# holo-routing/holo

Measured on NVIDIA H100. Metric: SPF recomputations/sec (10k-node LSDB), higher is better.
Workload: dtype u32

## Files before the change

holo_b200/csrc/spf_quad.cuh:

```cuda
#pragma once
#include <cstdint>
#include <cuda_runtime.h>

#include "spf_kernel.cuh"

namespace hspf {

constexpr uint32_t kJsInvalid = 8u;
constexpr uint32_t kJsInternal = 16u;
constexpr uint32_t kJsNarrow = 32u;
constexpr int kQMaxRoot = 64;

struct QuadDev {
    uint32_t NQ, NIQ, shift, isteps;
    const uint4 *fq;
    const uint32_t *fcont;
    const uint16_t *slot_of;
    const uint16_t *vert_of;
    const uint4 *iq;
    const uint2 *imeta;
    const uint32_t *fpos;
    const uint32_t *ipos;
};

struct QuadLayout {
    uint32_t dist, queue, ring, cont, h0, ecmp, elist, total;
    uint32_t qcap;
    uint32_t mhops;
    uint32_t mcap;
};

struct QuadArgs {
    DevGraph g;
    QuadDev q;
    QuadLayout lay;
    uint32_t n_jobs;
    const uint32_t *roots;
    const uint32_t *ov_off;
    const uint32_t *ov_edge;
    const uint32_t *ov_cost;
    uint32_t *out_dist;
    uint16_t *out_hops;
    uint32_t *out_fp;
    uint16_t *out_npar;
    uint64_t *out_nh;
    uint32_t *out_status;
    uint32_t *job_counter;
    uint32_t sub_rounds;
    uint32_t narrow;
    uint32_t n_peers;
    long long peer_delta[7];
    uint32_t *done;
    uint32_t done_chunk;
    unsigned long long *prof;
};

inline QuadLayout make_quad_layout(uint32_t V, uint32_t NQ, uint32_t qcap, uint32_t threads) {
    QuadLayout L{};
    auto al = [](size_t x) { return (uint32_t)((x + 15) / 16 * 16); };
    const uint32_t nbv = (V + 31) / 32, nbw = (NQ / 32 + 1u) & ~1u;
    const uint32_t Vp = (V + 4 * threads - 1) / (4 * threads) * (4 * threads);
    uint32_t o = 0;
    L.dist = o; o += al((size_t)NQ * 4);
    L.queue = o; o += al((size_t)qcap * 4);
    L.elist = al((size_t)Vp * 4);
    if (L.elist + al((size_t)V * 2) > o) o = L.elist + al((size_t)V * 2);
    L.ring = o; o += al((size_t)4 * nbw * 4);
    L.cont = o; o += al((size_t)nbw * 4);
    L.h0 = o; o += al((size_t)nbv * 4);
    L.ecmp = o; o += al((size_t)nbv * 4);
    L.total = o;
    L.qcap = qcap;
    if (L.cont >= L.elist + al((size_t)Vp * 2)) {
        L.mhops = L.cont - Vp * 2;
        L.mcap = (L.mhops - L.elist) / 2;
    }
    return L;
}

constexpr uint32_t kQuadThreads = 512;
constexpr uint32_t kQuadQcap = 2048;

inline size_t quad_smem_bytes(const QuadLayout &L) { return (size_t)L.total + 2048; }

struct QSmall {
    uint32_t cnt[2];
    uint32_t wake;
    uint32_t status;
    uint32_t job;
    uint32_t n_ov, sh;
    uint32_t ov_edge[kMaxOv], ov_cost[kMaxOv];
    uint32_t ov_fq[kMaxOv], ov_iq[kMaxOv];
    uint32_t n_roottab, root_rb, n_atoms;
    uint32_t mbad;
    uint16_t seed_of[16];
    uint32_t rt_target[kQMaxRoot], rt_base[kQMaxRoot], rt_cost[kQMaxRoot];
};

#define HSPF_QMARK(k)                                                            \
    do {                                                                         \
        if (a.prof && tid == 0) {                                                \
            const long long now_ = clock64();                                    \
            a.prof[(size_t)blockIdx.x * 16 + (k)] += (unsigned long long)(now_ - t_mark); \
            t_mark = now_;                                                       \
        }                                                                        \
    } while (0)

template <int T, bool kOv>
__global__ void __launch_bounds__(T, 3) spf_quad_kernel(const QuadArgs a) {
    extern __shared__ __align__(16) uint8_t qsm[];
    __shared__ QSmall S;

    const DevGraph &g = a.g;
    const QuadDev &Q = a.q;
    const QuadLayout &L = a.lay;
    const uint32_t V = g.V, NQ = Q.NQ, NBW = NQ >> 5, nbv = (V + 31) >> 5;
    const uint32_t NBWp = (NBW + 1u) & ~1u;
    const uint32_t tid = threadIdx.x, lane = tid & 31;
    const uint32_t qcap = L.qcap;

    uint32_t *dist = reinterpret_cast<uint32_t *>(qsm + L.dist);
    uint32_t *queue = reinterpret_cast<uint32_t *>(qsm + L.queue);
    uint32_t *ring = reinterpret_cast<uint32_t *>(qsm + L.ring);
    uint32_t *cont_s = reinterpret_cast<uint32_t *>(qsm + L.cont);
    uint32_t *h0bm = reinterpret_cast<uint32_t *>(qsm + L.h0);
    uint32_t *ecmpbm = reinterpret_cast<uint32_t *>(qsm + L.ecmp);
    uint32_t *word = dist;
    uint16_t *elist = reinterpret_cast<uint16_t *>(qsm + L.elist);

    long long t_mark = clock64();

    for (uint32_t w = tid; w < NBWp; w += T) cont_s[w] = (w < NBW) ? Q.fcont[w] : 0u;
    auto is_hop = [&](uint32_t v) -> bool { return (__ldg(&g.vflags[v]) & kVfHop) != 0; };
    const uint32_t Vp = (V + 4 * T - 1) / (4 * T) * (4 * T);
    const uint32_t U = g.reject_above + 1u ? g.reject_above + 1u : kInf;

    for (;;) {
        __syncthreads();
        if (tid == 0) S.job = atomicAdd(a.job_counter, 1u);
        __syncthreads();
        const uint32_t job = S.job;
        if (job >= a.n_jobs) break;
        const uint32_t root = a.roots[job];
        uint32_t n_ov_raw = 0;
        if (kOv && a.ov_off) n_ov_raw = a.ov_off[job + 1] - a.ov_off[job];
        if (root >= V || n_ov_raw > (uint32_t)kMaxOv) {
            if (tid == 0) {
                a.out_status[job] = kJsInvalid;
                for (uint32_t k = 0; k < (a.narrow ? a.n_peers : 0u); ++k)
                    *reinterpret_cast<uint32_t *>(reinterpret_cast<char *>(&a.out_status[job]) + a.peer_delta[k]) = kJsInvalid;
                if (a.done) { __threadfence(); atomicAdd(&a.done[job / a.done_chunk], 1u); }
            }
            continue;
        }
        const size_t jo = (size_t)job * V;
        const bool narrow = a.narrow != 0;
        uint32_t *o_dist = a.out_dist + jo;
        uint16_t *o_hops = a.out_hops + jo;
        uint32_t *o_fp = a.out_fp + jo;
        uint16_t *o_npar = a.out_npar + jo;
        uint64_t *o_nh = a.out_nh + jo;
        uint16_t *o_dist16 = reinterpret_cast<uint16_t *>(a.out_dist) + jo;
        uint16_t *o_fp16 = reinterpret_cast<uint16_t *>(a.out_fp) + jo;
        uint16_t *o_nh16 = reinterpret_cast<uint16_t *>(a.out_nh) + jo;
        const uint32_t n_peers = narrow ? a.n_peers : 0u;
        auto peer_push_row = [&](uint16_t *row) {
            char *src = reinterpret_cast<char *>(row);
            const size_t bytes = (size_t)V * 2;
            const size_t head = (16 - (reinterpret_cast<uintptr_t>(src) & 15)) & 15;
            const size_t h = head < bytes ? head : bytes;
            const size_t n16 = (bytes - h) / 16, tail0 = h + n16 * 16;
            for (size_t i = tid; i < n16; i += T) {
                const uint4 val = __ldcg(reinterpret_cast<const uint4 *>(src + h) + i);
                for (uint32_t k = 0; k < n_peers; ++k)
                    reinterpret_cast<uint4 *>(src + h + a.peer_delta[k])[i] = val;
            }
            auto push16 = [&](size_t o) {
                const uint16_t val = __ldcg(reinterpret_cast<const uint16_t *>(src + o));
                for (uint32_t k = 0; k < n_peers; ++k) *reinterpret_cast<uint16_t *>(src + o + a.peer_delta[k]) = val;
            };
            for (size_t o = (size_t)tid * 2; o < h; o += (size_t)T * 2) push16(o);
            for (size_t o = tail0 + (size_t)tid * 2; o < bytes; o += (size_t)T * 2) push16(o);
        };
        auto ld_fp = [&](uint32_t v) -> uint32_t {
            if (narrow) { const uint32_t f = __ldcg(&o_fp16[v]); return f == 0xFFFFu ? kInf : f; }
            return __ldcg(&o_fp[v]);
        };
        auto ld_dist = [&](uint32_t v) -> uint32_t {
            if (narrow) { const uint32_t d = __ldcg(&o_dist16[v]); return d == 0xFFFFu ? kInf : d; }
            return __ldcg(&o_dist[v]);
        };

        {
            uint4 *d4 = reinterpret_cast<uint4 *>(dist);
            const uint4 inf4 = make_uint4(U, U, U, U);
            for (uint32_t i = tid; i < NQ / 4; i += T) d4[i] = inf4;
            for (uint32_t i = tid; i < 4 * NBWp; i += T) ring[i] = 0;
            for (uint32_t w = tid; w < nbv; w += T) { h0bm[w] = 0; ecmpbm[w] = 0; }
        }
        if (tid == 0) {
            S.status = 0;
            S.cnt[0] = 0;
            S.cnt[1] = 0;
            S.wake = 0;
            S.n_ov = n_ov_raw;
            S.sh = Q.shift;
        }
        __syncthreads();
        if (kOv && tid < n_ov_raw) {
            const uint32_t e = a.ov_edge[a.ov_off[job] + tid];
            const uint32_t c = a.ov_cost[a.ov_off[job] + tid];
            if (e >= g.E) {
                atomicOr(&S.status, kJsInvalid);
                S.ov_edge[tid] = kInf; S.ov_cost[tid] = kInf; S.ov_fq[tid] = kInf; S.ov_iq[tid] = kInf;
            } else {
                S.ov_edge[tid] = e;
                S.ov_cost[tid] = c;
                S.ov_fq[tid] = Q.fpos[e];
                S.ov_iq[tid] = Q.ipos[e];
                const uint32_t tail = Q.vert_of[Q.fpos[e] >> 2];
                if (c == 0 && (g.vflags[tail] & kVfHop)) atomicOr(&S.status, kJsOrder);
                if (c != kInf) {
                    uint32_t sh = Q.shift;
                    while (sh < 31 && (3ull << sh) < (unsigned long long)c) ++sh;
                    atomicMax(&S.sh, sh);
                }
            }
        }
        const uint32_t rs = Q.slot_of[root];
        if (tid == 0) {
            dist[rs] = 0;
            ring[(rs >> 5) << 2] = 1u << (rs & 31);
        }
        __syncthreads();
        const uint32_t n_ov = kOv ? S.n_ov : 0u;
        auto ov_cost_of = [&](uint32_t e, uint32_t c) -> uint32_t {
            for (uint32_t k = 0; k < n_ov; ++k)
                if (S.ov_edge[k] == e) c = S.ov_cost[k];
            return c;
        };
        if (tid == 32 % T) {
            const uint32_t rb = g.row[root], re = g.row[root + 1];
            uint32_t nt = 0, nextbase = re - rb;
            for (uint32_t e = rb; e < re; ++e) {
                const uint2 ec = g.edge[e];
                const uint32_t h = ec.x;
                if (!(g.vflags[h] & kVfHop)) {
                    if (nt < (uint32_t)kQMaxRoot) {
                        S.rt_target[nt] = h;
                        S.rt_base[nt] = nextbase;
                        S.rt_cost[nt] = ov_cost_of(e, ec.y);
                        ++nt;
                    } else {
                        atomicOr(&S.status, kJsTooManyAtoms);
                    }
                    nextbase += g.row[h + 1] - g.row[h];
                }
            }
            S.n_roottab = nt;
            S.root_rb = rb;
            if (nextbase > 64u) { atomicOr(&S.status, kJsTooManyAtoms); nextbase = 64u; }
            S.n_atoms = nextbase;
        }
        __syncthreads();
        HSPF_QMARK(0);

        const uint32_t sh = kOv ? S.sh : Q.shift;
        {
            auto relax = [&](uint32_t q, uint32_t first, uint32_t du, const uint4 &r4) {
                uint32_t hs[4] = {r4.x & 0xFFFFu, r4.y & 0xFFFFu, r4.z & 0xFFFFu, r4.w & 0xFFFFu};
                uint32_t cs[4] = {r4.x >> 16, r4.y >> 16, r4.z >> 16, r4.w >> 16};
                if (kOv) {
                    for (uint32_t k = 0; k < n_ov; ++k) {
                        const uint32_t fp_ = S.ov_fq[k];
                        if ((fp_ >> 2) != q) continue;
                        const uint32_t c = S.ov_cost[k];
#pragma unroll
                        for (int j = 0; j < 4; ++j)
                            if ((fp_ & 3u) == (uint32_t)j) {
                                if (c == kInf) { hs[j] = first; cs[j] = 0xFFFFu; } else cs[j] = c;
                            }
                    }
                }
                uint32_t dh[4];
#pragma unroll
                for (int j = 0; j < 4; ++j) dh[j] = dist[hs[j]];
#pragma unroll
                for (int j = 0; j < 4; ++j) {
                    const uint32_t nd = kOv ? sat_add(du, cs[j]) : du + cs[j];
                    if (nd < dh[j]) {
                        const uint32_t old = atomicMin(&dist[hs[j]], nd);
                        if (old > nd) atomicOr(&ring[((hs[j] >> 5) << 2) + ((nd >> sh) & 3u)], 1u << (hs[j] & 31));
                    }
                }
            };
            constexpr uint32_t kWarps_ = T / 32;
            const uint32_t warp = tid >> 5;
            const uint32_t cw = min(32u, (NBWp + kWarps_ - 1) / kWarps_);
            const uint32_t nchunks = (NBWp + cw - 1) / cw;
            const uint32_t sub_rounds = a.sub_rounds;
            auto pick = [&](uint32_t t, uint32_t incl, uint32_t bits, uint32_t meta, uint32_t C) -> uint32_t {
                uint32_t lo = 0;
#pragma unroll
                for (uint32_t step = 16; step >= 1; step >>= 1) {
                    const uint32_t v = __shfl_sync(0xffffffffu, incl, lo + step - 1);
                    if (v <= t) lo += step;
                }
                lo &= 31u;
                const uint32_t ob = __shfl_sync(0xffffffffu, bits, lo);
                const uint32_t om = __shfl_sync(0xffffffffu, meta, lo);
                const uint32_t oc = __shfl_sync(0xffffffffu, C, lo);
                uint32_t k = t - (om & 0xFFFFu), pos = 0, cc;
                cc = __popc(ob & 0xFFFFu); if (k >= cc) { k -= cc; pos = 16; }
                cc = __popc((ob >> pos) & 0xFFu); if (k >= cc) { k -= cc; pos += 8; }
                cc = __popc((ob >> pos) & 0xFu); if (k >= cc) { k -= cc; pos += 4; }
                cc = __popc((ob >> pos) & 0x3u); if (k >= cc) { k -= cc; pos += 2; }
                cc = (ob >> pos) & 1u; if (k >= cc) pos += 1;
                pos &= 31u;
                const uint32_t fb = 31u - __clz((~oc & ((2u << pos) - 1u)) | 1u);
                const uint32_t qb = (om >> 16) * 32;
                return (qb + pos) | ((qb + fb) << 16);
            };
            uint32_t cur = 0, empties = 0;
            bool bucket_work = false;
            for (uint32_t guard = 0;; ++guard) {
                if (guard > (1u << 24)) { if (tid == 0) atomicOr(&S.status, kJsInternal); break; }
                uint32_t *bm = ring + (cur & 3u);
                int claimed = 0;
                for (uint32_t sr = 0; sr < sub_rounds; ++sr) {
                    for (uint32_t c = warp; c < nchunks; c += kWarps_) {
                        const uint32_t w = c * cw + lane;
                        const bool mine = lane < cw && w < NBWp;
                        uint32_t bits = mine ? *reinterpret_cast<volatile uint32_t *>(&bm[w << 2]) : 0u;
                        if (!__any_sync(0xffffffffu, bits != 0)) continue;
                        claimed = 1;
                        uint32_t C = 0;
                        if (bits) {
                            bits = atomicExch(&bm[w << 2], 0u);
                            C = cont_s[w];
                            uint32_t m = bits;
                            while ((m = (m << 1) & C) != 0) bits |= m;
                        }
                        const uint32_t cnt = __popc(bits);
                        uint32_t incl = cnt;
#pragma unroll
                        for (int o = 1; o < 32; o <<= 1) {
                            const uint32_t t = __shfl_up_sync(0xffffffffu, incl, o);
                            if ((int)lane >= o) incl += t;
                        }
                        const uint32_t n = __shfl_sync(0xffffffffu, incl, 31);
                        const uint32_t meta = (incl - cnt) | (w << 16);
                        if (a.prof && lane == 0) atomicAdd(&a.prof[(size_t)blockIdx.x * 16 + 12], (unsigned long long)n);
                        for (uint32_t t0 = 0; t0 < n; t0 += 64) {
                            const uint32_t ta = t0 + lane, tb = ta + 32;
                            const bool hb = t0 + 32 < n;
                            const uint32_t e0 = pick(ta, incl, bits, meta, C);
                            const uint32_t e1 = hb ? pick(tb, incl, bits, meta, C) : 0u;
                            const uint32_t du0 = (ta < n) ? dist[e0 >> 16] : kInf;
                            const uint32_t du1 = (hb && tb < n) ? dist[e1 >> 16] : kInf;
                            const bool l0 = (du0 >> sh) == cur, l1 = (du1 >> sh) == cur;
                            uint4 r0 = make_uint4(0u, 0u, 0u, 0u), r1 = r0;
                            if (l0) r0 = __ldg(&Q.fq[e0 & 0xFFFFu]);
                            if (l1) r1 = __ldg(&Q.fq[e1 & 0xFFFFu]);
                            if (l0) relax(e0 & 0xFFFFu, e0 >> 16, du0, r0);
                            if (l1) relax(e1 & 0xFFFFu, e1 >> 16, du1, r1);
                        }
                    }
                }
                if (a.prof && tid == 0) a.prof[(size_t)blockIdx.x * 16 + 7] += 1;
                if (__syncthreads_or(claimed)) { bucket_work = true; continue; }
                if (bucket_work) empties = 0;
                else if (++empties == 4) break;
                bucket_work = false;
                ++cur;
            }
        }
        HSPF_QMARK(1);

        if (tid < S.n_roottab) {
            const uint32_t h = S.rt_target[tid], c = S.rt_cost[tid];
            if (c < U && dist[Q.slot_of[h]] == c) atomicOr(&h0bm[h >> 5], 1u << (h & 31));
        }
        __syncthreads();
        auto hops0 = [&](uint32_t u) -> bool { return u == root || ((h0bm[u >> 5] >> (u & 31)) & 1u); };

        const uint32_t n_atoms = S.n_atoms;
        uint32_t seed_v = kInf;
        if (tid < n_atoms) {
            const uint32_t atom = tid, rdeg = g.row[root + 1] - S.root_rb;
            uint32_t e = kInf, u = root;
            if (atom < rdeg) {
                e = S.root_rb + atom;
            } else {
                for (uint32_t k = 0; k < S.n_roottab; ++k) {
                    const uint32_t N = S.rt_target[k], nb = S.rt_base[k];
                    if (atom < nb || atom >= nb + (g.row[N + 1] - g.row[N])) continue;
                    bool first = true;
                    for (uint32_t q = 0; q < k; ++q) first = first && S.rt_target[q] != N;
                    if (first && hops0(N)) { u = N; e = g.row[N] + (atom - nb); }
                    break;
                }
            }
            if (e != kInf) {
                const uint2 ec = g.edge[e];
                const uint32_t c = kOv ? ov_cost_of(e, ec.y) : ec.y;
                const uint32_t du = dist[Q.slot_of[u]], dh = dist[Q.slot_of[ec.x]];
                if (du < U && dh < U && c != kInf && sat_add(du, c) == dh &&
                    !((g.flags & kGfNoHopTargetNoNh) && !is_hop(ec.x)))
                    seed_v = ec.x;
            }
        }

        {
            uint32_t sat_flag = 0, narrow_flag = 0;
            const uint32_t NIQ = Q.NIQ, isteps = Q.isteps;
            auto pull = [&](uint32_t i, const uint2 &m, const uint4 &r4, uint32_t &dv, uint32_t &cnt, uint32_t &bd, uint32_t &bs) {
                const uint32_t sv = (m.x != 0xFFFFFFFFu) ? (m.x & 0xFFFFu) : 0u;
                dv = dist[sv];
                uint32_t su[4] = {r4.x & 0xFFFFu, r4.y & 0xFFFFu, r4.z & 0xFFFFu, r4.w & 0xFFFFu};
                uint32_t cs[4] = {r4.x >> 16, r4.y >> 16, r4.z >> 16, r4.w >> 16};
                if (kOv) {
                    for (uint32_t k = 0; k < n_ov; ++k) {
                        const uint32_t ip_ = S.ov_iq[k];
                        if ((ip_ >> 2) != i) continue;
                        const uint32_t c = S.ov_cost[k];
#pragma unroll
                        for (int j = 0; j < 4; ++j)
                            if ((ip_ & 3u) == (uint32_t)j) {
                                if (c == kInf) { su[j] = sv; cs[j] = 0xFFFFu; } else cs[j] = c;
                            }
                    }
                }
                uint32_t du[4];
#pragma unroll
                for (int j = 0; j < 4; ++j) du[j] = dist[su[j]];
                cnt = 0; bd = kInf; bs = kInf;
#pragma unroll
                for (int j = 0; j < 4; ++j) {
                    const uint32_t nd = kOv ? sat_add(du[j], cs[j]) : du[j] + cs[j];
                    const bool ok = du[j] < U && nd == dv;
                    const bool better = ok && (du[j] < bd || (du[j] == bd && su[j] < bs));
                    cnt += ok ? 1u : 0u;
                    bd = better ? du[j] : bd;
                    bs = better ? su[j] : bs;
                }
            };
            auto combine = [&](uint32_t rem, uint32_t &cnt, uint32_t &bd, uint32_t &bs) {
                for (uint32_t s = 0, d = 1; s < isteps; ++s, d <<= 1) {
                    const uint32_t ocnt = __shfl_down_sync(0xffffffffu, cnt, d);
                    const uint32_t obd = __shfl_down_sync(0xffffffffu, bd, d);
                    const uint32_t obs = __shfl_down_sync(0xffffffffu, bs, d);
                    if (d <= rem) {
                        cnt += ocnt;
                        if (obd < bd || (obd == bd && obs < bs)) { bd = obd; bs = obs; }
                    }
                }
            };
            auto emit_v = [&](const uint2 &m, uint32_t dv, uint32_t cnt, uint32_t bs) {
                if (m.x != 0xFFFFFFFFu && ((m.y >> 8) & 0xFFu) == 0) {
                    const uint32_t v = m.x >> 16;
                    if (dv >= U) dv = kInf;
                    if (v == root || dv == kInf) { cnt = 0; bs = kInf; }
                    if (dv != kInf && g.saturate_at && dv >= g.saturate_at) sat_flag = 1;
                    const uint32_t fpv = cnt ? (uint32_t)__ldg(&Q.vert_of[bs]) : kInf;
                    if (narrow) {
                        if (dv != kInf && dv >= 0xFFFFu) narrow_flag = 1;
                        o_dist16[v] = (uint16_t)min(dv, 0xFFFFu);
                        o_fp16[v] = (uint16_t)min(fpv, 0xFFFFu);

                    } else {
                        o_dist[v] = dv;
                        o_fp[v] = fpv;
                    }
                    o_npar[v] = (uint16_t)min(cnt, 0xFFFFu);
                    if (cnt >= 2) atomicOr(&ecmpbm[v >> 5], 1u << (v & 31));
                }
            };
            const uint32_t wbase = tid & ~31u;
            for (uint32_t i0 = 0; i0 + wbase < NIQ; i0 += 2 * T) {
                const uint32_t ia = i0 + tid, ib = ia + T;
                const bool hb = i0 + T + wbase < NIQ;
                const uint2 ma = __ldg(&Q.imeta[ia]);
                const uint4 ra = __ldg(&Q.iq[ia]);
                uint2 mb = make_uint2(0xFFFFFFFFu, 0u);
                uint4 rb = make_uint4(0u, 0u, 0u, 0u);
                if (hb) { mb = __ldg(&Q.imeta[ib]); rb = __ldg(&Q.iq[ib]); }
                uint32_t dva, ca, bda, bsa, dvb = kInf, cb = 0, bdb = kInf, bsb = kInf;
                pull(ia, ma, ra, dva, ca, bda, bsa);
                if (hb) pull(ib, mb, rb, dvb, cb, bdb, bsb);
                combine(ma.y & 0xFFu, ca, bda, bsa);
                if (hb) combine(mb.y & 0xFFu, cb, bdb, bsb);
                emit_v(ma, dva, ca, bsa);
                if (hb) emit_v(mb, dvb, cb, bsb);
            }
            if (sat_flag) atomicOr(&S.status, kJsSaturated);
            if (narrow_flag) atomicOr(&S.status, kJsNarrow);
        }
        __syncthreads();
        HSPF_QMARK(2);

        auto is_ecmp = [&](uint32_t v) -> bool { return (ecmpbm[v >> 5] >> (v & 31)) & 1u; };
        if (tid == 0) S.cnt[0] = 0;
        __syncthreads();
        for (uint32_t w0 = 0; w0 < nbv; w0 += T) {
            const uint32_t w = w0 + tid;
            const uint32_t bits = (w < nbv) ? ecmpbm[w] : 0u;
            if (!__any_sync(0xffffffffu, bits != 0)) continue;
            const uint32_t n = __popc(bits);
            uint32_t incl = n;
#pragma unroll
            for (int o = 1; o < 32; o <<= 1) {
                const uint32_t t = __shfl_up_sync(0xffffffffu, incl, o);
                if ((int)lane >= o) incl += t;
            }
            const uint32_t tot = __shfl_sync(0xffffffffu, incl, 31);
            uint32_t base = 0;
            if (lane == 31) base = atomicAdd(&S.cnt[0], tot);
            base = __shfl_sync(0xffffffffu, base, 31);
            uint32_t pos = base + incl - n;
            for (uint32_t b = bits; b; b &= b - 1) elist[pos++] = (uint16_t)(w * 32 + (__ffs(b) - 1));
        }
        __syncthreads();
        const uint32_t n_e = S.cnt[0];
        auto parents = [&](uint32_t x, auto &&f) {
            const uint32_t dx = ld_dist(x);
            for (uint32_t j = g.irow[x]; j < g.irow[x + 1]; ++j) {
                uint32_t u, c;
                if constexpr (kOv) {
                    const uint4 r = g.iedge[j];
                    u = r.x; c = ov_cost_of(r.z, r.y);
                    if (c == kInf) continue;
                } else {
                    const uint32_t r = g.iedge16[j];
                    u = r & 0xFFFFu; c = r >> 16;
                }
                const uint32_t du = ld_dist(u);
                if (du != kInf && sat_add(du, c) == dx && !hops0(u)) f(u);
            }
        };
        uint32_t pc[4] = {kInf, kInf, kInf, kInf};
        bool cached = false;
        if (n_e <= (uint32_t)T && tid < n_e) {
            uint32_t n = 0;
            parents(elist[tid], [&](uint32_t u) {
#pragma unroll
                for (int k = 0; k < 4; ++k) if (n == (uint32_t)k) pc[k] = u;
                ++n;
            });
            cached = n <= 4;
        }
        bool merged = L.mhops != 0 && n_atoms <= 12u && n_e <= L.mcap;
        if (merged) {
            const uint32_t na = n_atoms;
            uint32_t ovf = 0;
            for (uint32_t v = tid; v < Vp; v += T) {
                uint32_t A = v, h = 0;
                if (v < V && !is_ecmp(v)) {
                    const uint32_t f = ld_fp(v);
                    if (f != kInf) {
                        h = is_hop(v) ? 1u : 0u;
                        A = f;
                        if (hops0(f)) {
                            A = root;
                            for (uint32_t u = f, k = 0; u != root && u < V && k < V; u = ld_fp(u), ++k)
                                h += is_hop(u) ? 1u : 0u;
                        }
                    }
                }
                ovf |= h << na;
                word[v] = (A << 16) | ((h << na) & 0xFFFFu);
            }
            if (tid < 16u) S.seed_of[tid] = (uint16_t)min(seed_v, 0xFFFFu);
            if (tid == 0) S.mbad = 0;
            __syncthreads();
            if (seed_v != kInf && seed_v == root) ovf |= 1u << 16;
            else if (seed_v != kInf && !is_ecmp(seed_v)) atomicOr(&word[seed_v], 1u << tid);
            __syncthreads();
            for (uint32_t rounds = 0;;) {
                uint32_t moved = 0;
                for (uint32_t v0 = tid; v0 < Vp; v0 += 4 * T) {
                    uint32_t w[4], w2[4], w3[4];
#pragma unroll
                    for (int k = 0; k < 4; ++k) w[k] = word[v0 + k * T];
#pragma unroll
                    for (int k = 0; k < 4; ++k) w2[k] = word[w[k] >> 16];
#pragma unroll
                    for (int k = 0; k < 4; ++k) w3[k] = word[w2[k] >> 16];
#pragma unroll
                    for (int k = 0; k < 4; ++k) {
                        const uint32_t sum = (w[k] & 0xFFFFu) + (w2[k] & 0xFFFFu) + (w3[k] & 0xFFFFu);
                        ovf |= sum;
                        word[v0 + k * T] = (w3[k] & 0xFFFF0000u) | (sum & 0xFFFFu);
                        moved |= w3[k] ^ w[k];
                    }
                }
                if (ovf >> 16) S.mbad = 1;
                if (a.prof && tid == 0) a.prof[(size_t)blockIdx.x * 16 + 14] += 1;
                if (!__syncthreads_or((moved >> 16) != 0)) break;
                if (++rounds > 32u) { if (tid == 0) atomicOr(&S.status, kJsInternal); break; }
            }
            merged = S.mbad == 0;
            HSPF_QMARK(5);
        }
        if (merged) {
            const uint32_t na = n_atoms, amask = (1u << na) - 1u;
            uint16_t *eh = reinterpret_cast<uint16_t *>(qsm + L.mhops);
            if (n_e) {
                uint32_t fx = kInf;
                for (uint32_t i = tid; i < n_e; i += T) {
                    const uint32_t x = elist[i];
                    const uint32_t f = ld_fp(x);
                    fx = f;
                    uint32_t seeds = 0;
                    for (uint32_t b = 0; b < na; ++b) seeds |= (S.seed_of[b] == x) ? 1u << b : 0u;
                    uint32_t nw;
                    if (hops0(f)) nw = (root << 16) | seeds;
                    else if (is_ecmp(f)) nw = (f << 16) | seeds;
                    else { const uint32_t wf = word[f]; nw = (wf & 0xFFFF0000u) | ((wf | seeds) & amask); }
                    word[x] = nw;
                    eh[x] = 0xFFFFu;
                }
                __syncthreads();
                for (uint32_t sweeps = 0;;) {
                    int ch = 0;
                    for (uint32_t i = tid; i < n_e; i += T) {
                        const uint32_t x = elist[i];
                        const uint32_t w = word[x], Tx = w >> 16;
                        uint32_t need = (Tx != root) ? word[Tx] : 0u;
                        auto pull_parent = [&](uint32_t u) {
                            const uint32_t wp = word[u], Tp = wp >> 16;
                            need |= wp;
                            if (Tp != root && Tp != u) need |= word[Tp];
                        };
                        if (cached) {
#pragma unroll
                            for (int k = 0; k < 4; ++k) if (pc[k] != kInf) pull_parent(pc[k]);
                        } else {
                            parents(x, pull_parent);
                        }
                        need &= amask & ~w;
                        if (need) { word[x] = w | need; ch = 1; }
                        if (eh[x] == 0xFFFFu) {
                            const uint32_t f = (n_e <= (uint32_t)T) ? fx : ld_fp(x);
                            uint32_t h = is_hop(x) ? 1u : 0u, t = root;
                            if (is_ecmp(f)) t = f;
                            else if (f != root) { const uint32_t wf = word[f]; h += (wf & 0xFFFFu) >> na; t = wf >> 16; }
                            const uint32_t ht = (t == root) ? 0u : eh[t];
                            if (ht != 0xFFFFu) { eh[x] = (uint16_t)(h + ht); ch = 1; }
                        }
                    }
                    if (a.prof && tid == 0) a.prof[(size_t)blockIdx.x * 16 + 15] += 1;
                    if (!__syncthreads_or(ch)) break;
                    if (++sweeps > 17u * n_e + 16u) { if (tid == 0) atomicOr(&S.status, kJsInternal); break; }
                }
            }
            for (uint32_t v = tid; v < V; v += T) {
                const uint32_t w = word[v], Tv = w >> 16;
                const bool up = Tv != root && Tv != v;
                uint32_t m = w & amask, h;
                if (up) m |= word[Tv] & amask;
                if (is_ecmp(v)) h = eh[v];
                else h = ((w & 0xFFFFu) >> na) + (up ? (uint32_t)eh[Tv] : 0u);
                h &= 0xFFFFu;
                o_hops[v] = (uint16_t)h;
                if (h == 0 && v != root && Tv != v && !hops0(v) && g.row[v + 1] != g.row[v])
                    atomicOr(&S.status, kJsTooManyAtoms);
                if (narrow) o_nh16[v] = (uint16_t)m;
                else o_nh[v] = m;
            }
            __syncthreads();
        } else {
            for (uint32_t v = tid; v < Vp; v += T) {
                const uint32_t f = (v < V) ? ld_fp(v) : kInf;
                word[v] = (f == kInf) ? (v << 16) : ((f << 16) | (is_hop(v) ? 1u : 0u));
            }
            __syncthreads();
            uint32_t jump_rounds = 0;
            for (;;) {
                uint32_t moved = 0;
                for (uint32_t v0 = tid; v0 < Vp; v0 += 4 * T) {
                    uint32_t w[4], w2[4], w3[4];
    #pragma unroll
                    for (int k = 0; k < 4; ++k) w[k] = word[v0 + k * T];
    #pragma unroll
                    for (int k = 0; k < 4; ++k) w2[k] = word[w[k] >> 16];
    #pragma unroll
                    for (int k = 0; k < 4; ++k) w3[k] = word[w2[k] >> 16];
    #pragma unroll
                    for (int k = 0; k < 4; ++k) {
                        word[v0 + k * T] = (w3[k] & 0xFFFF0000u) | ((w[k] + w2[k] + w3[k]) & 0xFFFFu);
                        moved |= w3[k] ^ w[k];
                    }
                }
                if (a.prof && tid == 0) a.prof[(size_t)blockIdx.x * 16 + 13] += 1;
                if (!__syncthreads_or((moved >> 16) != 0)) break;
                if (++jump_rounds > 32u) { if (tid == 0) atomicOr(&S.status, kJsInternal); break; }
            }
            for (uint32_t v = tid; v < V; v += T) {
                const uint32_t w = word[v];
                const uint32_t h = (w >> 16) == v ? 0u : (w & 0xFFFFu);
                o_hops[v] = (uint16_t)h;
                if (h == 0 && v != root && (w >> 16) != v && !hops0(v) && g.row[v + 1] != g.row[v])
                    atomicOr(&S.status, kJsTooManyAtoms);
            }
            __syncthreads();
            HSPF_QMARK(5);

            for (uint32_t pass = 0; pass * 16u < n_atoms || pass == 0; ++pass) {
                for (uint32_t v = tid; v < Vp; v += T) {
                    uint32_t A = v;
                    if (v < V) {
                        const uint32_t f = ld_fp(v);
                        if (f != kInf && !is_ecmp(v)) A = hops0(f) ? root : f;
                    }
                    word[v] = A << 16;
                }
                __syncthreads();
                if (seed_v != kInf && (tid >> 4) == pass) atomicOr(&word[seed_v], 1u << (tid & 15));
                __syncthreads();
                for (uint32_t r = 0; r < jump_rounds; ++r) {
                    for (uint32_t v0 = tid; v0 < Vp; v0 += 4 * T) {
                        uint32_t w[4], w2[4], w3[4];
    #pragma unroll
                        for (int k = 0; k < 4; ++k) w[k] = word[v0 + k * T];
    #pragma unroll
                        for (int k = 0; k < 4; ++k) w2[k] = word[w[k] >> 16];
    #pragma unroll
                        for (int k = 0; k < 4; ++k) w3[k] = word[w2[k] >> 16];
    #pragma unroll
                        for (int k = 0; k < 4; ++k)
                            word[v0 + k * T] = (w3[k] & 0xFFFF0000u) | ((w[k] | w2[k] | w3[k]) & 0xFFFFu);
                    }
                    if (a.prof && tid == 0) a.prof[(size_t)blockIdx.x * 16 + 14] += 1;
                    __syncthreads();
                }
                if (n_e) {
                    for (uint32_t i = tid; i < n_e; i += T) {
                        const uint32_t x = elist[i];
                        const uint32_t seeds = word[x] & 0xFFFFu;
                        const uint32_t f = ld_fp(x);
                        uint32_t nw;
                        if (hops0(f)) nw = (root << 16) | seeds;
                        else if (is_ecmp(f)) nw = (f << 16) | seeds;
                        else { const uint32_t wf = word[f]; nw = (wf & 0xFFFF0000u) | ((wf | seeds) & 0xFFFFu); }
                        word[x] = nw;
                    }
                    __syncthreads();
                    for (uint32_t sweeps = 0;;) {
                        int ch = 0;
                        for (uint32_t i = tid; i < n_e; i += T) {
                            const uint32_t x = elist[i];
                            const uint32_t w = word[x], Tx = w >> 16;
                            uint32_t need = (Tx != root) ? word[Tx] : 0u;
                            auto pull_parent = [&](uint32_t u) {
                                const uint32_t wp = word[u], Tp = wp >> 16;
                                need |= wp;
                                if (Tp != root && Tp != u) need |= word[Tp];
                            };
                            if (cached) {
    #pragma unroll
                                for (int k = 0; k < 4; ++k) if (pc[k] != kInf) pull_parent(pc[k]);
                            } else {
                                parents(x, pull_parent);
                            }
                            need &= 0xFFFFu & ~w;
                            if (need) { word[x] = w | need; ch = 1; }
                        }
                        if (a.prof && tid == 0) a.prof[(size_t)blockIdx.x * 16 + 15] += 1;
                        if (!__syncthreads_or(ch)) break;
                        if (++sweeps > 16u * n_e + 16u) { if (tid == 0) atomicOr(&S.status, kJsInternal); break; }
                    }
                }
                for (uint32_t v = tid; v < V; v += T) {
                    const uint32_t w = word[v], Tv = w >> 16;
                    uint32_t m = w;
                    if (Tv != root && Tv != v) m |= word[Tv];
                    if (narrow) {
                        if (pass == 0) {
                            o_nh16[v] = (uint16_t)(m & 0xFFFFu);
                        }
                    } else {
                        const uint64_t bits = (uint64_t)(m & 0xFFFFu) << (16 * pass);
                        if (pass == 0) o_nh[v] = bits; else o_nh[v] |= bits;
                    }
                }
                __syncthreads();
            }
        }
        if (n_peers) {
            __syncthreads();
            peer_push_row(o_dist16);
            peer_push_row(o_hops);
            peer_push_row(o_nh16);
        }
        if (tid == 0) {
            const uint32_t st = S.status | ((narrow && n_atoms > 16u) ? kJsNarrow : 0u);
            a.out_status[job] = st;
            for (uint32_t k = 0; k < n_peers; ++k)
                *reinterpret_cast<uint32_t *>(reinterpret_cast<char *>(&a.out_status[job]) + a.peer_delta[k]) = st;
        }
        if (a.done) {
            __syncthreads();
            if (tid == 0) { __threadfence(); atomicAdd(&a.done[job / a.done_chunk], 1u); }
        }
        HSPF_QMARK(4);
    }
}

__global__ void patch_costs_kernel(DevGraph g, QuadDev q, bool has_quads, uint32_t n, const uint32_t *edges,
                                   const uint32_t *costs) {
    const uint32_t i = blockIdx.x * blockDim.x + threadIdx.x;
    if (i >= n) return;
    const uint32_t e = edges[i], c = costs[i];
    uint2 *edge = const_cast<uint2 *>(g.edge);
    const uint32_t v = edge[e].x;
    edge[e].y = c;
    if (g.edge16) const_cast<uint32_t *>(g.edge16)[e] = v | (c << 16);
    uint4 *iedge = const_cast<uint4 *>(g.iedge);
    for (uint32_t k = g.irow[v]; k < g.irow[v + 1]; ++k) {
        if (iedge[k].z != e) continue;
        iedge[k].y = c;
        if (g.iedge16) {
            const uint32_t rec = iedge[k].x | (c << 16);
            const_cast<uint32_t *>(g.iedge16)[k] = rec;
            if (g.iquad) reinterpret_cast<uint32_t *>(const_cast<uint4 *>(g.iquad))[(size_t)g.iquad_row[v] * 4 + (k - g.irow[v])] = rec;
        }
        break;
    }
    if (has_quads) {
        uint32_t *fq = reinterpret_cast<uint32_t *>(const_cast<uint4 *>(q.fq));
        uint32_t *iq = reinterpret_cast<uint32_t *>(const_cast<uint4 *>(q.iq));
        const uint32_t fp = q.fpos[e], ip = q.ipos[e];
        fq[fp] = (fq[fp] & 0xFFFFu) | (c << 16);
        iq[ip] = (iq[ip] & 0xFFFFu) | (c << 16);
    }
}

}
```

Before: 1.893 million.

## Derive vertex IDs from shared rank table and batch fp loads across phases

Replaces the per-vertex global gather of vert_of with a per-32-slot base table staged in shared memory (reusing the ring buffer) plus a popcount over the continuation bitmask. Restructures the interior pull loop for the non-overlap variant into a single-stride loop with software prefetch of the next imeta/iq entries. Unrolls the word-initialisation loops in the merged and jump paths by four so the ld_fp loads are issued together before use. The changes aim to cut global-load latency in post-SPF processing, at the cost of relying on ring being free and cont_s being valid at that point.

```diff
diff --git a/holo_b200/csrc/spf_quad.cuh b/holo_b200/csrc/spf_quad.cuh
--- a/holo_b200/csrc/spf_quad.cuh
+++ b/holo_b200/csrc/spf_quad.cuh
@@ -377,6 +377,8 @@
         }
         HSPF_QMARK(1);
 
+        uint16_t *vbase = reinterpret_cast<uint16_t *>(ring);
+        for (uint32_t w = tid; w < NBW; w += T) vbase[w] = __ldg(&Q.vert_of[w << 5]);
         if (tid < S.n_roottab) {
             const uint32_t h = S.rt_target[tid], c = S.rt_cost[tid];
             if (c < U && dist[Q.slot_of[h]] == c) atomicOr(&h0bm[h >> 5], 1u << (h & 31));
@@ -462,7 +464,7 @@
                     if (dv >= U) dv = kInf;
                     if (v == root || dv == kInf) { cnt = 0; bs = kInf; }
                     if (dv != kInf && g.saturate_at && dv >= g.saturate_at) sat_flag = 1;
-                    const uint32_t fpv = cnt ? (uint32_t)__ldg(&Q.vert_of[bs]) : kInf;
+                    const uint32_t fpv = cnt ? vbase[bs >> 5] + __popc(~cont_s[bs >> 5] & ((1u << (bs & 31)) - 1u)) : kInf;
                     if (narrow) {
                         if (dv != kInf && dv >= 0xFFFFu) narrow_flag = 1;
                         o_dist16[v] = (uint16_t)min(dv, 0xFFFFu);
@@ -477,21 +479,35 @@
                 }
             };
             const uint32_t wbase = tid & ~31u;
-            for (uint32_t i0 = 0; i0 + wbase < NIQ; i0 += 2 * T) {
-                const uint32_t ia = i0 + tid, ib = ia + T;
-                const bool hb = i0 + T + wbase < NIQ;
-                const uint2 ma = __ldg(&Q.imeta[ia]);
-                const uint4 ra = __ldg(&Q.iq[ia]);
-                uint2 mb = make_uint2(0xFFFFFFFFu, 0u);
-                uint4 rb = make_uint4(0u, 0u, 0u, 0u);
-                if (hb) { mb = __ldg(&Q.imeta[ib]); rb = __ldg(&Q.iq[ib]); }
-                uint32_t dva, ca, bda, bsa, dvb = kInf, cb = 0, bdb = kInf, bsb = kInf;
-                pull(ia, ma, ra, dva, ca, bda, bsa);
-                if (hb) pull(ib, mb, rb, dvb, cb, bdb, bsb);
-                combine(ma.y & 0xFFu, ca, bda, bsa);
-                if (hb) combine(mb.y & 0xFFu, cb, bdb, bsb);
-                emit_v(ma, dva, ca, bsa);
-                if (hb) emit_v(mb, dvb, cb, bsb);
+            if constexpr (!kOv) {
+                uint2 nm = make_uint2(0xFFFFFFFFu, 0u);
+                uint4 nr = make_uint4(0u, 0u, 0u, 0u);
+                if (wbase < NIQ) { nm = __ldg(&Q.imeta[tid]); nr = __ldg(&Q.iq[tid]); }
+                for (uint32_t i = tid; i - lane < NIQ; i += T) {
+                    const uint2 m = nm;
+                    uint32_t dv, cnt, bd, bs;
+                    pull(i, m, nr, dv, cnt, bd, bs);
+                    if (i + T - lane < NIQ) { nm = __ldg(&Q.imeta[i + T]); nr = __ldg(&Q.iq[i + T]); }
+                    combine(m.y & 0xFFu, cnt, bd, bs);
+                    emit_v(m, dv, cnt, bs);
+                }
+            } else {
+                for (uint32_t i0 = 0; i0 + wbase < NIQ; i0 += 2 * T) {
+                    const uint32_t ia = i0 + tid, ib = ia + T;
+                    const bool hb = i0 + T + wbase < NIQ;
+                    const uint2 ma = __ldg(&Q.imeta[ia]);
+                    const uint4 ra = __ldg(&Q.iq[ia]);
+                    uint2 mb = make_uint2(0xFFFFFFFFu, 0u);
+                    uint4 rb = make_uint4(0u, 0u, 0u, 0u);
+                    if (hb) { mb = __ldg(&Q.imeta[ib]); rb = __ldg(&Q.iq[ib]); }
+                    uint32_t dva, ca, bda, bsa, dvb = kInf, cb = 0, bdb = kInf, bsb = kInf;
+                    pull(ia, ma, ra, dva, ca, bda, bsa);
+                    if (hb) pull(ib, mb, rb, dvb, cb, bdb, bsb);
+                    combine(ma.y & 0xFFu, ca, bda, bsa);
+                    if (hb) combine(mb.y & 0xFFu, cb, bdb, bsb);
+                    emit_v(ma, dva, ca, bsa);
+                    if (hb) emit_v(mb, dvb, cb, bsb);
+                }
             }
             if (sat_flag) atomicOr(&S.status, kJsSaturated);
             if (narrow_flag) atomicOr(&S.status, kJsNarrow);
@@ -553,22 +569,29 @@
         if (merged) {
             const uint32_t na = n_atoms;
             uint32_t ovf = 0;
-            for (uint32_t v = tid; v < Vp; v += T) {
-                uint32_t A = v, h = 0;
-                if (v < V && !is_ecmp(v)) {
-                    const uint32_t f = ld_fp(v);
+            for (uint32_t v0 = tid; v0 < Vp; v0 += 4 * T) {
+                uint32_t fk[4];
+#pragma unroll
+                for (int k = 0; k < 4; ++k) {
+                    const uint32_t v = v0 + k * T;
+                    fk[k] = (v < V && !is_ecmp(v)) ? ld_fp(v) : kInf;
+                }
+#pragma unroll
+                for (int k = 0; k < 4; ++k) {
+                    const uint32_t v = v0 + k * T, f = fk[k];
+                    uint32_t A = v, h = 0;
                     if (f != kInf) {
                         h = is_hop(v) ? 1u : 0u;
                         A = f;
                         if (hops0(f)) {
                             A = root;
-                            for (uint32_t u = f, k = 0; u != root && u < V && k < V; u = ld_fp(u), ++k)
+                            for (uint32_t u = f, n = 0; u != root && u < V && n < V; u = ld_fp(u), ++n)
                                 h += is_hop(u) ? 1u : 0u;
                         }
                     }
-                }
-                ovf |= h << na;
-                word[v] = (A << 16) | ((h << na) & 0xFFFFu);
+                    ovf |= h << na;
+                    word[v] = (A << 16) | ((h << na) & 0xFFFFu);
+                }
             }
             if (tid < 16u) S.seed_of[tid] = (uint16_t)min(seed_v, 0xFFFFu);
             if (tid == 0) S.mbad = 0;
@@ -670,9 +693,15 @@
             }
             __syncthreads();
         } else {
-            for (uint32_t v = tid; v < Vp; v += T) {
-                const uint32_t f = (v < V) ? ld_fp(v) : kInf;
-                word[v] = (f == kInf) ? (v << 16) : ((f << 16) | (is_hop(v) ? 1u : 0u));
+            for (uint32_t v0 = tid; v0 < Vp; v0 += 4 * T) {
+                uint32_t fk[4];
+#pragma unroll
+                for (int k = 0; k < 4; ++k) fk[k] = (v0 + k * T < V) ? ld_fp(v0 + k * T) : kInf;
+#pragma unroll
+                for (int k = 0; k < 4; ++k) {
+                    const uint32_t v = v0 + k * T;
+                    word[v] = (fk[k] == kInf) ? (v << 16) : ((fk[k] << 16) | (is_hop(v) ? 1u : 0u));
+                }
             }
             __syncthreads();
             uint32_t jump_rounds = 0;
@@ -707,13 +736,16 @@
             HSPF_QMARK(5);
 
             for (uint32_t pass = 0; pass * 16u < n_atoms || pass == 0; ++pass) {
-                for (uint32_t v = tid; v < Vp; v += T) {
-                    uint32_t A = v;
-                    if (v < V) {
-                        const uint32_t f = ld_fp(v);
-                        if (f != kInf && !is_ecmp(v)) A = hops0(f) ? root : f;
-                    }
-                    word[v] = A << 16;
+                for (uint32_t v0 = tid; v0 < Vp; v0 += 4 * T) {
+                    uint32_t fk[4];
+#pragma unroll
+                    for (int k = 0; k < 4; ++k) fk[k] = (v0 + k * T < V) ? ld_fp(v0 + k * T) : kInf;
+#pragma unroll
+                    for (int k = 0; k < 4; ++k) {
+                        const uint32_t v = v0 + k * T, f = fk[k];
+                        const uint32_t A = (f != kInf && !is_ecmp(v)) ? (hops0(f) ? root : f) : v;
+                        word[v] = A << 16;
+                    }
                 }
                 __syncthreads();
                 if (seed_v != kInf && (tid >> 4) == pass) atomicOr(&word[seed_v], 1u << (tid & 15));
```

Result: faster. 1.963 million, median of 6 (+3.7%).
